# frgfm/Holocron

Measured on AMD Instinct MI355X. Metric: images/sec fwd+bwd+AdaBelief, RepVGG-A0 bs256/GPU 224^2, higher is better.
Workload: dtype bf16; 1 GPU; repvgg_a0 bf16 train step (fwd+bwd+AdaBelief), synthetic 224^2, bs=256 per MI355X (BASELINE.json configs[1]), random-init weights, 10 classes, CE label_smoothing 0.1; global_batch=256, parallelism=dp1, mode=weight gradients on a second stream; hipGraph replay of the full step, dump_outputs=/tmp/code/gt15__hip_graft__frgfm__Holocron/driver_out/dump_parent, deterministic=True

## Files before the change

holocron_amd/_lib.py:

```python
import ctypes as C
import os

import torch

_HERE = os.path.dirname(os.path.abspath(__file__))
LIB_PATH = os.environ.get("HC_LIB_PATH") or os.path.join(_HERE, "lib", "libholocron_hip.so")

HC_MAX_TAPS = 12
HC_MT_CHUNK = 8192
HC_STAT_REPLICAS = 128

c_void_p, c_int32, c_int64, c_float, c_double = C.c_void_p, C.c_int32, C.c_int64, C.c_float, C.c_double


class ConvClass(C.Structure):
    _fields_ = [("OHg", c_int32), ("OWg", c_int32), ("oy0", c_int32), ("ox0", c_int32), ("ostep", c_int32),
                ("istep", c_int32), ("ntaps", c_int32), ("tap", c_int32 * HC_MAX_TAPS)]


class ConvDesc(C.Structure):
    _fields_ = [("src0", c_void_p), ("src1", c_void_p), ("wpk", c_void_p), ("dst", c_void_p), ("resid", c_void_p),
                ("stats", c_void_p), ("bias", c_void_p), ("act", c_int32),
                ("N", c_int32), ("IH", c_int32), ("IW", c_int32), ("srcC", c_int32),
                ("OH", c_int32), ("OW", c_int32), ("Cout", c_int32), ("T", c_int32), ("nclass", c_int32),
# ... 160 lines not shown
    "hc_space_to_depth": (c_int32, [c_void_p] * 2 + [c_int32] * 8 + [c_void_p]),
    "hc_leaky_bwd": (c_int32, [c_void_p, c_int32, c_void_p, c_void_p, c_int64, c_int32, c_float, c_void_p]),
    "hc_yolo1_loss_fwd": (c_int32, [c_void_p] * 3 + [c_int32] * 8 + [c_void_p] * 4 + [c_int32] + [c_void_p] * 4),
    "hc_yolo1_loss_bwd": (c_int32, [c_void_p] * 3 + [c_int32] * 8 + [c_void_p] * 4 + [c_int32] + [c_void_p] * 7),
    "hc_yolo1_decode": (c_int32, [c_void_p] * 3 + [c_int32] * 7 + [c_void_p] * 4),
    "hc_yolo_format_fwd": (c_int32, [c_void_p] * 2 + [c_int32] * 7 + [c_void_p] * 5),
    "hc_yolo_format_bwd": (c_int32, [c_void_p] * 3 + [c_int32] * 7 + [c_void_p] * 7),
    "hc_lamb_step": (c_int32, [c_void_p, c_int32, c_void_p, c_void_p, c_void_p, c_int32, c_void_p]),
    "hc_tadam_step": (c_int32, [c_void_p, c_int32, c_void_p, c_void_p, c_void_p, c_void_p, c_void_p, c_void_p, c_int32, c_void_p]),
    "hc_adan_step": (c_int32, [c_void_p, c_void_p, c_int32, c_void_p, c_void_p]),
    "hc_lookahead_sync": (c_int32, [c_void_p, c_int32, c_float, c_void_p]),
    "hc_multi_copy": (c_int32, [C.POINTER(MultiCopyDesc), c_void_p]),
    "hc_msbn_finalize": (c_int32, [C.POINTER(MsbnDesc), c_void_p]),
    "hc_msbn_bwd_finalize": (c_int32, [C.POINTER(MsbnDesc), c_void_p]),
    "hc_msbn_apply": (c_int32, [C.POINTER(MsbnIo), c_void_p, c_void_p, c_void_p, c_int32, c_void_p]),
    "hc_msbn_bwd_reduce": (c_int32, [C.POINTER(MsbnIo), c_void_p, c_int32, c_void_p, c_void_p, c_int32, c_void_p]),
    "hc_msbn_bwd_apply": (c_int32, [C.POINTER(MsbnIo), c_void_p, c_int32, c_void_p, c_void_p, c_int32, c_void_p]),
    "hc_dwrep_dgrad": (c_int32, [c_void_p, c_void_p, c_int32, c_void_p, c_void_p] + [c_int32] * 5 + [c_void_p]),
    "hc_conv_gather": (c_int32, [C.POINTER(ConvDesc), c_void_p]),
    "hc_conv_pointwise_supported": (c_int32, [C.POINTER(ConvDesc)]),
    "hc_conv_pointwise": (c_int32, [C.POINTER(ConvDesc), c_void_p]),
    "hc_conv_small": (c_int32, [C.POINTER(ConvSmallDesc), c_void_p]),
    "hc_conv_small_supported": (c_int32, [C.POINTER(ConvSmallDesc)]),
    "hc_conv_s2_supported": (c_int32, [C.POINTER(ConvS2Desc)]),
    "hc_conv_s2_fwd": (c_int32, [C.POINTER(ConvS2Desc), c_void_p]),
    "hc_conv_s2_dgrad_supported": (c_int32, [C.POINTER(ConvS2DgradDesc)]),
    "hc_conv_s2_dgrad": (c_int32, [C.POINTER(ConvS2DgradDesc), c_void_p]),
    "hc_conv_s2_stem_wgrad_ws_bytes": (c_int64, []),
    "hc_conv_s2_stem_wgrad": (c_int32, [c_void_p] * 6 + [c_int32] * 4 + [c_void_p]),
    "hc_conv_wgrad_ws_bytes": (c_int64, [C.POINTER(WgradDesc)]),
    "hc_conv_wgrad": (c_int32, [C.POINTER(WgradDesc), c_void_p]),
    "hc_conv_wgrad_group_supported": (c_int32, [C.POINTER(WgradGroupDesc)]),
    "hc_conv_wgrad_group_ws_bytes": (c_int64, [C.POINTER(WgradGroupDesc)]),
    "hc_conv_wgrad_group": (c_int32, [C.POINTER(WgradGroupDesc), c_void_p]),
    "hc_rep_wgrad_supported": (c_int32, [C.POINTER(RepWgradDesc)]),
    "hc_rep_wgrad_ws_bytes": (c_int64, [C.POINTER(RepWgradDesc)]),
    "hc_rep_wgrad_plan": (c_int32, [C.POINTER(RepWgradDesc), c_void_p]),
    "hc_rep_wgrad": (c_int32, [C.POINTER(RepWgradDesc), c_void_p]),
    "hc_pack_conv_weight": (c_int32, [c_void_p, c_void_p] + [c_int32] * 7 + [c_void_p]),
    "hc_pack_conv_weights_multi": (c_int32, [c_void_p, c_int32, c_int64, c_void_p]),
    "hc_nchw_to_nhwc_bf16": (c_int32, [c_void_p, c_void_p] + [c_int32] * 5 + [c_void_p]),
    "hc_nhwc_bf16_to_nchw": (c_int32, [c_void_p, c_void_p] + [c_int32] * 5 + [c_void_p]),
    "hc_im2col_small": (c_int32, [c_void_p, c_void_p] + [c_int32] * 11 + [c_void_p]),
    "hc_unpack_im2col_grad": (c_int32, [c_void_p, c_void_p] + [c_int32] * 6 + [c_void_p]),
    "hc_rep_bn_finalize": (c_int32, [C.POINTER(RepBnDesc), c_void_p]),
    "hc_rep_apply": (c_int32, [c_void_p] * 6 + [c_int64, c_int32, c_int32, c_void_p]),
# ... 152 lines not shown
```

holocron_amd/build.py:

```python
import os
import subprocess
import sys
from concurrent.futures import ThreadPoolExecutor

ROOT = os.path.dirname(os.path.abspath(__file__))
CSRC = os.path.join(ROOT, "csrc")
LIBDIR = os.path.join(ROOT, "lib")
LIB = os.path.join(LIBDIR, "libholocron_hip.so")
HIPCC = os.environ.get("HIPCC", "/opt/rocm/bin/hipcc")
ARCH = "gfx950"

SOURCES = {
    "conv_gather.hip": ["-mllvm", "-pragma-unroll-threshold=131072"],
    "conv_pointwise.hip": [],
    "conv_small.hip": [],
    "conv_wgrad.hip": [],
    "conv_wgrad_tr.hip": [],
    "conv_wgrad_dma.hip": [],
    "conv_wgrad_rep.hip": [],
    "conv_rows.hip": [],
    "conv_rows48.hip": [],
    "conv_s2.hip": [],
    "rep_bn.hip": [],
    "optim.hip": [],
    "nhwc_ops.hip": [],
    "dwconv.hip": [],
    "se_mlp.hip": [],
    "mobileone.hip": [],
    "pointwise.hip": ["-ffp-contract=off"],
    "losses.hip": ["-ffp-contract=off"],
    "yolo.hip": ["-ffp-contract=off"],
}
COMMON = ["--offload-arch=" + ARCH, "-O3", "-std=c++17", "-fPIC", "-Wno-unused-result"]


def _deps():
    hdrs = [os.path.join(CSRC, "common.h"), os.path.join(ROOT, "..", "include", "holocron_hip.h")]
    return max(os.path.getmtime(h) for h in hdrs)


def _compile(item):
    src, flags = item
    obj = os.path.join(LIBDIR, src.replace(".hip", ".o"))
    srcp = os.path.join(CSRC, src)
    if os.path.exists(obj) and os.path.getmtime(obj) >= max(os.path.getmtime(srcp), _deps()):
        return obj, False
    cmd = [HIPCC] + COMMON + flags + ["-c", srcp, "-o", obj]
    r = subprocess.run(cmd, capture_output=True, text=True)
    if r.returncode != 0:
        raise RuntimeError("hipcc failed for %s:\n%s\n%s" % (src, r.stdout, r.stderr))
    return obj, True


def build(force: bool = False, verbose: bool = False) -> str:
    os.makedirs(LIBDIR, exist_ok=True)
    if force:
        for f in os.listdir(LIBDIR):
            if f.endswith(".o") or f.endswith(".so"):
                os.remove(os.path.join(LIBDIR, f))
    with ThreadPoolExecutor(max_workers=min(8, len(SOURCES))) as ex:
# ... 16 lines not shown
```

holocron_amd/csrc/conv_rows.hip:

```cpp
#include <type_traits>
#include "common.h"
#include "../../include/holocron_hip.h"

namespace crw {

constexpr int NT = 512, UR = 7;

struct Args {
    hc_conv_small_desc d;
    int reps;
    int delay;
};

template <int C, int W>
struct Geo {
    static constexpr int CK = C / 32;
    static constexpr int PSC = C / 8 + 1;
    static constexpr int PS = PSC * 16;
    static constexpr int SEGW = W > 0 ? (W + 15) / 16 : (C >= 192 ? 1 : 2);
    static constexpr int WMAX = W > 0 ? W : 16 * SEGW;
    static constexpr int WW = WMAX + 1;
    static constexpr int NSLOT = (UR + 2) * WW + 1;
    static constexpr int NDMA = (NSLOT * PS + 1023) / 1024;
    static constexpr int WIN = NDMA * 1024;
    static constexpr int CWN = 4 / SEGW;
    static constexpr int SMEM = 2 * WIN + 64 + 1024;
    static constexpr int S3 = 9 * CK, S1 = CK, S = S3 + S1;
    static_assert(C == 48 * CWN, "one wave = 48 output channels");
    static_assert(CK % 3 == 0, "three rotating weight register sets per tap");
    static_assert((PS / 8) % 4 == 2, "pixel pitch must be 2 x odd 8-byte units");
    static_assert(SMEM <= 160 * 1024, "LDS budget");
};

__device__ __forceinline__ void dma16s(const u32x4 rsrc, unsigned lds_off, unsigned voff, unsigned soff) {
    asm volatile("s_mov_b32 m0, %0\n\ts_nop 0\n\tbuffer_load_dwordx4 %1, %2, %3 offen lds" ::"s"(lds_off), "v"(voff), "s"(rsrc), "s"(soff)
                 : "memory");
}
__device__ __forceinline__ u32x4 uniform_rsrc(const void* p, unsigned bytes) {
    const unsigned long long v = reinterpret_cast<unsigned long long>(p);
    u32x4 r;
    r[0] = __builtin_amdgcn_readfirstlane((unsigned)v);
    r[1] = __builtin_amdgcn_readfirstlane((unsigned)(v >> 32) & 0xffffu);
    r[2] = __builtin_amdgcn_readfirstlane(bytes);
    r[3] = 0x00020000u;
    return r;
}
__device__ __forceinline__ bf16x8 frag2(const char* lo_p, const char* hi_p) {
    const u32x2 lo = *reinterpret_cast<const u32x2*>(lo_p), hi = *reinterpret_cast<const u32x2*>(hi_p);
    const u32x4 v = {lo[0], lo[1], hi[0], hi[1]};
    return __builtin_bit_cast(bf16x8, v);
}
__device__ __forceinline__ float row16_sum(float v) {
    v += __builtin_bit_cast(float, __builtin_amdgcn_update_dpp(0, __builtin_bit_cast(int, v), 0x128, 0xf, 0xf, false));
    v += __builtin_bit_cast(float, __builtin_amdgcn_update_dpp(0, __builtin_bit_cast(int, v), 0x124, 0xf, 0xf, false));
    v += __builtin_bit_cast(float, __builtin_amdgcn_update_dpp(0, __builtin_bit_cast(int, v), 0x122, 0xf, 0xf, false));
    v += __builtin_bit_cast(float, __builtin_amdgcn_update_dpp(0, __builtin_bit_cast(int, v), 0x121, 0xf, 0xf, false));
    return v;
}

template <int C, int W, int MODE, int DBG>
__global__ __launch_bounds__(NT, 1) void conv_rows_kernel(const Args a) {
    using G = Geo<C, W>;
    extern __shared__ __attribute__((aligned(1024))) char smem[];
    const hc_conv_small_desc& d = a.d;
    constexpr int CK = G::CK, PS = G::PS, WW = G::WW, S3 = G::S3, S1 = G::S1, S = G::S;
    const int tid = threadIdx.x, lane = tid & 63;
    const int wid = __builtin_amdgcn_readfirstlane(tid >> 6);
    const int team = wid >> 2, w4 = wid & 3;
    const int cw = w4 % G::CWN, pw = w4 / G::CWN;
    const int H = d.H, UPI = W > 0 ? H / UR : (H + UR - 1) / UR;
    const int Wr = W > 0 ? W : d.W;
    const int n = blockIdx.x;
    const unsigned lds0 = hc_lds_addr(smem);
    const int px = lane & 15, g = lane >> 4;
    const int col = 16 * pw + px;
    const bool col_ok = col < Wr;
    const int region = team * G::WIN;
    int* cnt = reinterpret_cast<int*>(smem + 2 * G::WIN) + team * 8;
    int gen = 0;
    if (tid < 16) reinterpret_cast<int*>(smem + 2 * G::WIN)[tid] = 0;
    __syncthreads();
    auto team_sync = [&]() __attribute__((always_inline)) {
        asm volatile("s_waitcnt vmcnt(0) lgkmcnt(0)" ::: "memory");
        gen += 4;
        if (lane == 0) __hip_atomic_fetch_add(cnt, 1, __ATOMIC_RELAXED, __HIP_MEMORY_SCOPE_WORKGROUP);
        while (__hip_atomic_load(cnt, __ATOMIC_RELAXED, __HIP_MEMORY_SCOPE_WORKGROUP) < gen) __builtin_amdgcn_s_sleep(1);
        asm volatile("" ::: "memory");
    };
    if (team == 1)
        for (int i = 0; i < a.delay; ++i) __builtin_amdgcn_s_sleep(64);

    const unsigned act_bytes = (unsigned)d.N * H * Wr * C * 2u;
    const u32x4 rsA = uniform_rsrc(d.srcA, act_bytes);
    const u32x4 rsB = uniform_rsrc(MODE == 1 ? d.srcB : d.srcA, act_bytes);
    const __amdgpu_buffer_rsrc_t rsw = make_rsrc(d.w3, (unsigned)(S * C * 64));

    const unsigned wl = (unsigned)((48 * cw + (lane & 15)) * 64 + g * 16);
    u32x4 af[3][3];
    auto load_a = [&](int buf, int s) __attribute__((always_inline)) {
        if (DBG & 4) return;
        const int ps = MODE == 0 ? (s < S1 ? S3 + s : s - S1) : s;
#pragma unroll
        for (int f = 0; f < 3; ++f) af[buf][f] = buf_load16(rsw, wl, (unsigned)(ps * (C * 64) + f * 1024));
    };

    auto stage_window = [&](const u32x4 rs, int row0, int j0, int j1) __attribute__((always_inline)) {
        if (DBG & 8) return;
        const unsigned img = (unsigned)n * (unsigned)(H * Wr * C * 2);
        for (int j = j0 + w4; j < j1; j += 4) {
            const int J = j * 64 + lane;
            const int slot = J / G::PSC, c = J - slot * G::PSC;
            const int r = slot / WW, x = slot - r * WW;
            const int ih = row0 - 1 + r;
            const bool ok = c < G::PSC - 1 && slot < G::NSLOT && x >= 1 && (W > 0 || x <= Wr) && ih >= 0 && ih < H;
            const unsigned off = img + (unsigned)((ih * Wr + x - 1) * C * 2 + c * 16);
            hc_dma16(rs, lds0 + (unsigned)(region + j * 1024), ok ? off : HC_OOB);
        }
    };

    const int vb = region + (WW + col + 1) * PS + g * 8;
    bf16x8 bfr[2][UR];
    auto load_b = [&](int buf, int bofs) __attribute__((always_inline)) {
        if (DBG & 2) return;
        const char* sb = smem + vb + bofs;
#pragma unroll
        for (int i = 0; i < UR; ++i) bfr[buf][i] = frag2(sb + i * WW * PS, sb + i * WW * PS + 32);
    };

    f32x4 acc[3][UR];
    auto zero_acc = [&]() __attribute__((always_inline)) {
#pragma unroll
        for (int f = 0; f < 3; ++f)
#pragma unroll
            for (int i = 0; i < UR; ++i) acc[f][i] = f32x4{0.f, 0.f, 0.f, 0.f};
    };
    auto mfma_step = [&](int ab, int bb) __attribute__((always_inline)) {
#pragma unroll
        for (int i = 0; i < UR; ++i)
#pragma unroll
// ... 36 lines not shown
        for (int k = 0; k < 2; ++k)
#pragma unroll
            for (int e = 0; e < 12; ++e) st[k][e] = 0.f;
#pragma unroll
        for (int i = 0; i < UR; ++i) {
            const bool ok = col_ok && (W > 0 || row0 + i < H);
            const int rr = W > 0 ? row0 + i : (ok ? row0 + i : 0);
            const size_t e0 = img + (size_t)(rr * Wr + (col_ok ? col : 0)) * C + cbase;
            bf16_t* op = reinterpret_cast<bf16_t*>(outp) + e0;
            const bf16_t* rp = residp != nullptr ? reinterpret_cast<const bf16_t*>(residp) + e0 : nullptr;
            u32x2 pk[3];
#pragma unroll
            for (int f = 0; f < 3; ++f) {
                f32x4 v = acc[f][i];
                const int cofs = f < 2 ? 4 * f : 32 - 4 * g;
                if (stats != nullptr) {
#pragma unroll
                    for (int e = 0; e < 4; ++e) {
                        const float x = ok ? v[e] : 0.f;
                        st[0][f * 4 + e] += x;
                        st[1][f * 4 + e] += x * x;
                    }
                }
                if (MODE == 1 && rp != nullptr && ok) {
                    const u32x2 rv = *reinterpret_cast<const u32x2*>(rp + cofs);
                    v[0] += bf16lo(rv[0]); v[1] += bf16hi(rv[0]); v[2] += bf16lo(rv[1]); v[3] += bf16hi(rv[1]);
                }
                pk[f] = u32x2{pack_bf16x2(v[0], v[1]), pack_bf16x2(v[2], v[3])};
                if (MODE == 1 && ok) *reinterpret_cast<u32x2*>(op + cofs) = pk[f];
            }
            if (MODE == 0 && ok) {
                *reinterpret_cast<u32x4*>(op) = u32x4{pk[0][0], pk[0][1], pk[1][0], pk[1][1]};
                *reinterpret_cast<u32x2*>(op + 32 - 4 * g) = pk[2];
            }
        }
        if (stats != nullptr) {
            float* rep = stats + (size_t)((blockIdx.x * 8 + wid) % a.reps) * 2 * C + cbase;
#pragma unroll
            for (int k = 0; k < 2; ++k) {
                float mine = 0.f;
#pragma unroll
                for (int e = 0; e < 12; ++e) {
                    const float x = row16_sum(st[k][e]);
                    mine = px == e ? x : mine;
                }
                if (px < 12) atomicAdd(rep + k * C + (px < 8 ? px : 24 - 4 * g + px), mine);
            }
        }
    };

    for (int u = team; u < UPI; u += 2) {
        const int row0 = u * UR;
        if (u >= 2) team_sync();
        stage_window(rsA, row0, 0, G::NDMA);
        team_sync();
        load_a(0, 0);
        load_a(1, 1);
        zero_acc();
        auto tap_ofs = [&](int tap) __attribute__((always_inline)) { return tap < 9 ? ((tap / 3 - 1) * WW + (tap % 3 - 1)) * PS : 0; };
        if (MODE == 0) {
            load_b(0, 0);
            tap_block(std::integral_constant<int, 0>{}, 0, S, 0, tap_ofs(0), true);
            epilogue(d.out1, d.stats1, nullptr, row0);
            zero_acc();
#pragma nounroll
            for (int tap = 0; tap < 8; tap += 2) {
                const int o0 = tap_ofs(tap), o1 = tap_ofs(tap + 1), o2 = tap_ofs(tap + 2);
                tap_block(std::integral_constant<int, (CK & 1)>{}, (tap + 1) * CK, S, o0, o1, true);
                tap_block(std::integral_constant<int, 0>{}, (tap + 2) * CK, S, o1, o2, true);
            }
            tap_block(std::integral_constant<int, (CK & 1)>{}, 9 * CK, S, tap_ofs(8), 0, false);
            epilogue(d.out3, d.stats3, nullptr, row0);
        } else {
            load_b(0, (-WW - 1) * PS);
#pragma nounroll
            for (int tap = 0; tap < 8; tap += 2) {
                const int o0 = tap_ofs(tap), o1 = tap_ofs(tap + 1), o2 = tap_ofs(tap + 2);
// ... 1 lines not shown
                tap_block(std::integral_constant<int, (CK & 1)>{}, (tap + 1) * CK, S, o1, o2, true);
            }
            tap_block(std::integral_constant<int, 0>{}, 8 * CK, S, tap_ofs(8), 0, false);
            team_sync();
            stage_window(rsB, row0, (WW * PS) / 1024, (8 * WW * PS + PS + 1023) / 1024);
            team_sync();
            load_b(S3 & 1, 0);
            tap_block(std::integral_constant<int, (S3 & 1)>{}, S3, S, 0, 0, false);
            epilogue(d.out3, nullptr, d.resid, row0);
        }
    }
}

template <int C, int W>
bool shape_ok(const hc_conv_small_desc& d) {
    if (W == 0)
        return d.C == C && d.Cout == C && d.W >= 1 && d.W <= Geo<C, 0>::WMAX && d.H >= 1 && d.N >= 1 &&
               (double)d.N * d.H * d.W * C * 2.0 < 2147483000.0;
    return d.C == C && d.Cout == C && d.W == W && d.H >= 2 * UR && d.H % (2 * UR) == 0 && d.H <= 56 && d.N >= 1 &&
           (double)d.N * d.H * d.W * C * 2.0 < 2147483000.0;
}

template <int C, int W, int MODE, int DBG>
void launch1(const Args& a, hipStream_t st) {
    auto kern = conv_rows_kernel<C, W, MODE, DBG>;
    constexpr int smem = Geo<C, W>::SMEM;
    static bool attr_set = false;
    if (!attr_set) {
        (void)hipFuncSetAttribute(reinterpret_cast<const void*>(kern), hipFuncAttributeMaxDynamicSharedMemorySize, smem);
        attr_set = true;
    }
    hipLaunchKernelGGL(kern, dim3(a.d.N), dim3(NT), smem, st, a);
}

template <int C, int W>
void launch(const Args& a, hipStream_t st) {
    static const int dbg = getenv("HC_CRW_DBG") ? atoi(getenv("HC_CRW_DBG")) : 0;
    const bool dg = (a.d.mode & 1) == 1;
#define CRW_CASE(k) case k: if (dg) launch1<C, W, 1, k>(a, st); else launch1<C, W, 0, k>(a, st); break;
    switch (dbg) {
        CRW_CASE(1) CRW_CASE(2) CRW_CASE(3) CRW_CASE(4) CRW_CASE(7) CRW_CASE(8) CRW_CASE(16) CRW_CASE(24) CRW_CASE(31)
        default: if (dg) launch1<C, W, 1, 0>(a, st); else launch1<C, W, 0, 0>(a, st); break;
    }
#undef CRW_CASE
}

}

bool hc_conv_rows_supported(const hc_conv_small_desc& d) {
    static const bool on = [] { const char* e = getenv("HC_CONV_ROWS"); return e == nullptr || atoi(e) != 0; }();
    if (!on || (d.mode & HC_CONV_SMALL_ROWS_IMAGE) == 0 || (d.mode & ~(HC_CONV_SMALL_ROWS_IMAGE | 1)) != 0) return false;
    constexpr bool any = true;
    if (crw::shape_ok<192, 14>(d) || crw::shape_ok<96, 28>(d)) return true;
    return any && (crw::shape_ok<192, 0>(d) || crw::shape_ok<96, 0>(d));
}
int hc_conv_rows_launch(const hc_conv_small_desc& d, hipStream_t st) {
    if (!hc_conv_rows_supported(d)) return HC_ERR_ARG;
    const bool dg = (d.mode & 1) == 1;
    if (d.srcA == nullptr || d.w3 == nullptr || d.out3 == nullptr) return HC_ERR_ARG;
    if (!dg && d.out1 == nullptr) return HC_ERR_ARG;
    if (dg && d.srcB == nullptr) return HC_ERR_ARG;
    if (!dg && (d.stats3 == nullptr) != (d.stats1 == nullptr)) return HC_ERR_ARG;
    crw::Args a;
    a.d = d;
    a.reps = hc_get_stat_replicas();
    constexpr int delay = 0;
    a.delay = delay;
    if (crw::shape_ok<192, 14>(d)) crw::launch<192, 14>(a, st);
    else if (crw::shape_ok<96, 28>(d)) crw::launch<96, 28>(a, st);
    else if (d.C == 192) { if (dg) crw::launch1<192, 0, 1, 0>(a, st); else crw::launch1<192, 0, 0, 0>(a, st); }
    else { if (dg) crw::launch1<96, 0, 1, 0>(a, st); else crw::launch1<96, 0, 0, 0>(a, st); }
    return hc_launch_status();
}
```

holocron_amd/csrc/rep_bn.hip:

```cpp
#include "common.h"
#include "../../include/holocron_hip.h"
#include <stdlib.h>

namespace {

constexpr int EW_THREADS = 256;

struct EwGrid {
    int blocks;
};
inline int ew_blocks(long nchunks, int cg, int cpt_default = 8) {
    int a = cg, b = EW_THREADS;
    while (b) { int t = a % b; a = b; b = t; }
    const int unit = cg / a;
    const int cpt = cpt_default;
    long want = nchunks / (EW_THREADS * cpt);
    constexpr long fl = 1024;
    long floor_blocks = nchunks / (EW_THREADS * 2);
    if (floor_blocks > fl) floor_blocks = fl;
    if (want < floor_blocks) want = floor_blocks;
    if (want > 2048) want = 2048;
    if (want < 1) want = 1;
    long k = (want + unit - 1) / unit;
    return (int)(k * unit);
}

__device__ __forceinline__ void unpack8(const u32x4 v, float (&f)[8]) {
#pragma unroll
    for (int i = 0; i < 4; ++i) { f[2 * i] = bf16lo(v[i]); f[2 * i + 1] = bf16hi(v[i]); }
}
__device__ __forceinline__ u32x4 pack8(const float (&f)[8]) {
    u32x4 v;
#pragma unroll
    for (int i = 0; i < 4; ++i) v[i] = pack_bf16x2(f[2 * i], f[2 * i + 1]);
    return v;
}
__device__ __forceinline__ void load8f(const float* p, float (&f)[8]) {
    const f32x4 a = *reinterpret_cast<const f32x4*>(p), b = *reinterpret_cast<const f32x4*>(p + 4);
#pragma unroll
    for (int i = 0; i < 4; ++i) { f[i] = a[i]; f[4 + i] = b[i]; }
}

template <bool NT>
__device__ __forceinline__ u32x4 ld16(const u32x4* p) {
    return NT ? __builtin_nontemporal_load(p) : *p;
}
template <bool NT>
__device__ __forceinline__ void st16(u32x4* p, const u32x4 v) {
    if (NT) __builtin_nontemporal_store(v, p);
    else *p = v;
}
static inline bool ba_streaming(long nchunks) { return nchunks * 16 >= 200L * 1000000L; }
static inline bool ew_streaming(long nchunks) {
    constexpr long thr = 48;
    return thr >= 0 && nchunks * 16 >= thr * 1000000L;
}

template <int S>
__device__ __forceinline__ void block_reduce_flush(const float (&v)[S][8], int cg, int C, float* __restrict__ dst,
                                                   float* __restrict__ lds, int nsum) {
    constexpr int STR = S * 8 + 1;
    const int tid = threadIdx.x;
#pragma unroll
    for (int k = 0; k < S; ++k)
#pragma unroll
// ... 87 lines not shown
                invstd = rsqrtf(var + d.eps);
                if (d.running_mean[b] != nullptr) {
                    const float unb = d.count > 1 ? var * (cnt / (cnt - 1.f)) : var;
                    d.running_mean[b][c] = (1.f - d.momentum) * rm[b] + d.momentum * mean;
                    d.running_var[b][c] = (1.f - d.momentum) * rv[b] + d.momentum * unb;
                }
                if (c == 0 && d.num_batches_tracked[b] != nullptr) d.num_batches_tracked[b][0] += 1;
            } else {
                mean = rm[b];
                invstd = rsqrtf(rv[b] + d.eps);
            }
            a = gam[b] * invstd;
            shift += bet[b] - a * mean;
        }
        d.coef[b * d.C + c] = a;
        if (d.save != nullptr) {
            d.save[(2 * b) * d.C + c] = mean;
            d.save[(2 * b + 1) * d.C + c] = invstd;
        }
    }
    d.coef[3 * d.C + c] = shift;
}

template <bool HAS_ID>
__device__ __forceinline__ float rep_preact(float a3, float f3, float a1, float f1, float a0, float f0, float sh) {
    float z = __builtin_fmaf(a1, f1, sh);
    if (HAS_ID) z = __builtin_fmaf(a0, f0, z);
    return __builtin_fmaf(a3, f3, z);
}
template <bool HAS_ID, bool STATS, bool NT>
__global__ __launch_bounds__(EW_THREADS) void rep_apply_kernel(const u32x4* __restrict__ y3, const u32x4* __restrict__ y1,
                                                               const u32x4* __restrict__ x, const float* __restrict__ coef,
                                                               u32x4* __restrict__ out, float* __restrict__ out_stats,
                                                               long nchunks, int C, int act, const int reps) {
    extern __shared__ float sred[];
    const int cg = C / 8;
    const long gtid = (long)blockIdx.x * EW_THREADS + threadIdx.x;
    const long stride = (long)gridDim.x * EW_THREADS;
    const int c0 = (int)(gtid % cg) * 8;
    float a3[8], a1[8], a0[8], sh[8];
    load8f(coef + c0, a3);
    load8f(coef + C + c0, a1);
    if (HAS_ID) load8f(coef + 2 * C + c0, a0);
    load8f(coef + 3 * C + c0, sh);
    float sv[2][8];
#pragma unroll
    for (int i = 0; i < 8; ++i) sv[0][i] = sv[1][i] = 0.f;
    for (long q = gtid; q < nchunks; q += stride) {
        float f3[8], f1[8], f0[8], o[8];
        unpack8(ld16<NT>(y3 + q), f3);
        unpack8(ld16<NT>(y1 + q), f1);
        if (HAS_ID) unpack8(ld16<NT>(x + q), f0);
// ... 169 lines not shown
    const long stride = (long)gridDim.x * EW_THREADS;
    const int c0 = (int)(gtid % cg) * 8;
    float a3[8], a1[8], a0[8], sh[8];
    if (ZMASK) {
        load8f(coef + c0, a3);
        load8f(coef + C + c0, a1);
        if (HAS_ID) load8f(coef + 2 * C + c0, a0);
        load8f(coef + 3 * C + c0, sh);
    }
    float A3[8], B3[8], C3[8], A1[8], B1[8], C1[8], A0[8], B0[8], C0[8];
    load8f(bc + 0 * C + c0, A3); load8f(bc + 1 * C + c0, B3); load8f(bc + 2 * C + c0, C3);
    load8f(bc + 3 * C + c0, A1); load8f(bc + 4 * C + c0, B1); load8f(bc + 5 * C + c0, C1);
    if (HAS_ID) { load8f(bc + 6 * C + c0, A0); load8f(bc + 7 * C + c0, B0); load8f(bc + 8 * C + c0, C0); }
    for (long q = gtid; q < nchunks; q += stride) {
        float fg[8], fo[8], f3[8], f1[8], f0[8], o3[8], o1[8], o0[8];
        unpack8(ld16<NT>(g + q), fg);
        if (!ZMASK) unpack8(ld16<NT>(out + q), fo);
        unpack8(ld16<NT>(y3 + q), f3);
        unpack8(ld16<NT>(y1 + q), f1);
        if (HAS_ID) unpack8(ld16<NT>(x + q), f0);
#pragma unroll
        for (int i = 0; i < 8; ++i) {
            if (ZMASK) fo[i] = act == 1 ? rep_preact<HAS_ID>(a3[i], f3[i], a1[i], f1[i], HAS_ID ? a0[i] : 0.f, HAS_ID ? f0[i] : 0.f, sh[i]) : 1.f;
            const float dz = fo[i] > 0.f ? fg[i] : 0.f;
            o3[i] = __builtin_fmaf(A3[i], dz, __builtin_fmaf(B3[i], f3[i], C3[i]));
            o1[i] = __builtin_fmaf(A1[i], dz, __builtin_fmaf(B1[i], f1[i], C1[i]));
            if (HAS_ID) o0[i] = __builtin_fmaf(A0[i], dz, __builtin_fmaf(B0[i], f0[i], C0[i]));
        }
        st16<NT>(dy3 + q, pack8(o3));
        st16<NT>(dy1 + q, pack8(o1));
        if (HAS_ID) st16<NT>(dxid + q, pack8(o0));
    }
}

__device__ __forceinline__ float act_fwd(float v, int act, float slope) {
    switch (act) {
        case 1: return v > 0.f ? v : 0.f;
        case 2: { const float t = fminf(fmaxf(v + 2.f, 0.f), 2.f); return 0.5f * v * t; }
        case 3: return v > 0.f ? v : slope * v;
        case 4: {
            const float e = __expf(fminf(v, 20.f)), n = e * (e + 2.f);
            return v * n * __builtin_amdgcn_rcpf(n + 2.f);
        }
        case 5: return v * __builtin_amdgcn_rcpf(1.f + __expf(-v));
        case 6: return fminf(fmaxf(v, 0.f), 6.f);
        default: return v;
    }
}
__device__ __forceinline__ float act_bwd(float v, int act, float slope) {
    switch (act) {
// ... 1030 lines not shown
```

holocron_amd/nn/repblock_op.py:

```python
import ctypes as C

import os

import torch

from .. import _lib
from .._lib import ConvS2Desc, ConvS2DgradDesc, PackItem, RepBnBwdDesc, RepBnDesc, StemBwdDesc, StemDesc, check, ptr, stream
from ..ops import conv as cv

STEM_KPAD = 32


class ZeroPool:

    def __init__(self):
        self.buf = None
        self.used = 0
        self.high = 0
        self.depth = 0
        self.gen = 0
        self.retired = []
        self.graph_users = 0
        self.buf_captured = False

    def _retire(self):
        if self.buf is not None and self.buf_captured:
            self.retired.append(self.buf)
        self.buf, self.buf_captured = None, False

    def release_retired(self):
        self.graph_users = max(0, self.graph_users - 1)
        if self.graph_users == 0:
            self.retired = []
# ... 294 lines not shown
    return y3, y1


def block_dgrad(st, dy3, dy1, dxid, w3, w1, geom):
    N, Cin, H, W, Cout = geom
    _, _, dg, _, sdg = st.descs(N, Cin, H, W, Cout)
    wpd = st.ensure_packed(w3, w1)[2]
    dx = cv.empty_cl(N, Cin, H, W, dy3.device)
    s2g = st.desc[(N, Cin, H, W, Cout)][7]
    if s2g is not None:
        if dxid is not None:
            raise _lib.HipError("stride-2 data gradient: a stride-2 RepBlock has no identity branch")
        s2g.dy3, s2g.dy1, s2g.wimg, s2g.dx = ptr(dy3), ptr(dy1), ptr(st.s2_dimg), ptr(dx)
        with cv.profiled("conv_s2", 2.0 * N * dy3.shape[2] * dy3.shape[3] * Cout * 10 * Cin, dx.numel() * 2.0 + 2 * dy3.numel() * 2.0):
            check(_lib.load().hc_conv_s2_dgrad(C.byref(s2g), stream()), "hc_conv_s2_dgrad")
        return dx
    if sdg is not None:
        cv.launch_conv_small_dgrad(sdg, dy3, dy1, wpd, dx, resid=dxid)
    else:
        cv.launch_conv(dg, dy3, wpd, dx, src1=dy1, resid=dxid)
    return dx


def block_wgrad(st, src, dy3, dy1, w3, w1, geom, stem_cin=None, defer=False):
    N, Cin, H, W, Cout = geom
    lib = _lib.load()
    npix = dy3.shape[0] * dy3.shape[2] * dy3.shape[3]
    if stem_cin is not None and src.dtype == torch.float32:
        dw3 = torch.empty_like(w3, dtype=torch.float32)
        dw1 = torch.empty_like(w1, dtype=torch.float32)
        ws = torch.empty((int(lib.hc_conv_s2_stem_wgrad_ws_bytes()),), dtype=torch.uint8, device=src.device)
        with cv.profiled("conv_wgrad", 2.0 * npix * Cout * 10 * stem_cin, src.numel() * 4.0 + 2 * dy3.numel() * 2.0):
            rc = lib.hc_conv_s2_stem_wgrad(ptr(src), ptr(dy3), ptr(dy1), ptr(dw3), ptr(dw1), ptr(ws), N, H, W, 0, stream())
        if rc == 0:
            return dw3, dw1
        src = cv.im2col_small(src, 3, 3, st.stride, 1, STEM_KPAD)
    if stem_cin is not None:
        K = STEM_KPAD
        dwc3 = cv.conv_wgrad(src, dy3, K, Cout, 1, 1, 1, 0, flops=2.0 * npix * Cout * 9 * stem_cin)
        dwc1 = cv.conv_wgrad(src, dy1, K, Cout, 1, 1, 1, 0, flops=2.0 * npix * Cout * stem_cin)
        dw3 = torch.empty_like(w3, dtype=torch.float32)
        check(lib.hc_unpack_im2col_grad(ptr(dwc3), ptr(dw3), Cout, stem_cin, 3, 3, K, 0, stream()), "hc_unpack_im2col_grad")
        dw1 = dwc1.view(Cout, K)[:, 4 * stem_cin:5 * stem_cin].reshape(Cout, stem_cin, 1, 1).contiguous()
        return dw3, dw1
    fused = cv.rep_block_wgrad(src, dy3, dy1, w3, w1, st.stride, defer=defer)
    if fused is not None:
# ... 132 lines not shown
            return (None, dw3, dw1, dgam[0], dbet[0], dgam[1], dbet[1], None, None, None, None)
        red = POOL.claim(ctx.red, ctx.red_gen, (_lib.stat_replicas(), 4, Cout), dev)
        ctx.red = None
        with cv.profiled("bn_elementwise", 0.0, tb * (4 if st.identity else 3)):
            check(lib.hc_rep_bwd_reduce_z(ptr(g), ptr(coef), act, ptr(y3), ptr(y1), ptr(xid), ptr(red), npix, Cout, stream()),
                  "hc_rep_bwd_reduce_z")
        nb = 3 if st.identity else 2
        dgam = torch.empty((3, Cout), dtype=torch.float32, device=dev)
        dbet = torch.empty((3, Cout), dtype=torch.float32, device=dev)
        bcoef = torch.empty((9, Cout), dtype=torch.float32, device=dev)
        d = RepBnBwdDesc()
        d.red, d.save, d.bcoef = ptr(red), ptr(save), ptr(bcoef)
        gam = (g3, g1, g0)
        for b in range(3):
            live = b < nb
            d.gamma[b] = ptr(gam[b]) if live else None
            d.dgamma[b] = ptr(dgam[b]) if live else None
            d.dbeta[b] = ptr(dbet[b]) if live else None
        d.C, d.count, d.has_identity, d.accumulate = Cout, npix, 1 if st.identity else 0, 0
        d.frozen = 0 if ctx.was_training else 1
        with cv.profiled("bn_finalize", 0.0, 0.0):
            check(lib.hc_rep_bn_bwd_finalize(C.byref(d), stream()), "hc_rep_bn_bwd_finalize")

        dy3 = torch.empty_like(y3)
        dy1 = torch.empty_like(y1)
        dxid = torch.empty_like(src) if st.identity else None
        with cv.profiled("bn_elementwise", 0.0, tb * (7 if st.identity else 5)):
            check(lib.hc_rep_bwd_apply_z(ptr(g), ptr(coef), act, ptr(y3), ptr(y1), ptr(xid), ptr(bcoef), ptr(dy3), ptr(dy1),
                                         ptr(dxid), npix, Cout, stream()), "hc_rep_bwd_apply_z")

        dx = None
        geom = (N, Cin, H, W, Cout)
        if ctx.needs_input_grad[0]:
            if ctx.stem:
                raise NotImplementedError("input gradient of the im2col stem path")
            dx = block_dgrad(st, dy3, dy1, dxid, w3, w1, geom)

        with cv.side_stream_for_wgrad((w3, w1), (src, dy3, dy1)) as side:
            dw3, dw1 = block_wgrad(st, src, dy3, dy1, w3, w1, geom, Cin if ctx.stem else None, defer=True)
            side.produced(dw3, dw1)
        return (dx, dw3, dw1, dgam[0], dbet[0], dgam[1], dbet[1],
                dgam[2] if st.identity else None, dbet[2] if st.identity else None, None, None)


def rep_block_forward(x, w3, w1, bn3, bn1, bn0, st, relu=True):
    st.bn = [(bn3.running_mean, bn3.running_var, bn3.num_batches_tracked),
             (bn1.running_mean, bn1.running_var, bn1.num_batches_tracked),
             (bn0.running_mean, bn0.running_var, bn0.num_batches_tracked) if bn0 is not None else (None, None, None)]
    st.eps = bn3.eps
    st.momentum = 0.1 if bn3.momentum is None else bn3.momentum
    st.training = bn3.training
    if bn1.training != bn3.training or (bn0 is not None and bn0.training != bn3.training):
        raise NotImplementedError("RepBlock (HIP): the BatchNorm layers of one block must all be in the same mode (freeze the "
                                  "whole block, e.g. freeze_model(model, 'features.2.1'), not a single branch)")
    out = RepBlockFn.apply(x, w3, w1, bn3.weight, bn3.bias, bn1.weight, bn1.bias,
                           bn0.weight if bn0 is not None else None, bn0.bias if bn0 is not None else None, st, relu)
    if st.last_out_stats is not None:
        out._hc_stats = st.last_out_stats
        st.last_out_stats = None
# ... 2 lines not shown
```

include/holocron_hip.h:

```cpp
#ifndef HOLOCRON_HIP_H
#define HOLOCRON_HIP_H
#include <stdint.h>
#ifdef __cplusplus
extern "C" {
#endif

typedef void* hc_stream_t;

#define HC_MAX_TAPS 12
#define HC_STAT_REPLICAS 128
#define HC_STAT_REPLICAS_DETERMINISTIC 32768
int hc_set_deterministic(int on);
int hc_get_deterministic(void);
int hc_get_stat_replicas(void);

typedef struct {
    int32_t OHg, OWg, oy0, ox0, ostep, istep, ntaps;
    int32_t tap[HC_MAX_TAPS];
} hc_conv_class;
#define HC_TAP(dy, dx, src, wt) \
    ((int32_t)(((uint32_t)(dy) & 0xffu) | (((uint32_t)(dx) & 0xffu) << 8) | ((uint32_t)(src) << 16) | ((uint32_t)(wt) << 24)))

typedef struct {
    const void* src0;
// ... 20 lines not shown
    float act_slope;
    int32_t resid_after_act;
} hc_conv_desc;
int hc_conv_gather(const hc_conv_desc* d, hc_stream_t stream);
int hc_conv_pointwise_supported(const hc_conv_desc* d);
int hc_conv_pointwise(const hc_conv_desc* d, hc_stream_t stream);

#define HC_CONV_SMALL_ROWS_IMAGE 4
typedef struct {
    const void* srcA;
    const void* srcB;
    const void* w3;
    const void* w1;
    void* out3;
    void* out1;
    const void* resid;
    float* stats3;
    float* stats1;
    int32_t w3_rstride, w1_rstride;
    int32_t N, H, W, C, Cout, mode;
} hc_conv_small_desc;
int hc_conv_small(const hc_conv_small_desc* d, hc_stream_t stream);
int hc_conv_small_supported(const hc_conv_small_desc* d);

typedef struct {
    const void* x;
    const void* w3img;
    const void* w1img;
    void* y3;
    void* y1;
    float* stats3;
    float* stats1;
    int32_t N, H, W, Cin, Cout, x_nchw_f32;
} hc_conv_s2_desc;
int hc_conv_s2_supported(const hc_conv_s2_desc* d);
int hc_conv_s2_fwd(const hc_conv_s2_desc* d, hc_stream_t stream);
typedef struct {
    const void* dy3;
    const void* dy1;
    const void* wimg;
    void* dx;
    int32_t N, H, W, Cin, Cout;
} hc_conv_s2_dgrad_desc;
int hc_conv_s2_dgrad_supported(const hc_conv_s2_dgrad_desc* d);
int hc_conv_s2_dgrad(const hc_conv_s2_dgrad_desc* d, hc_stream_t stream);
int64_t hc_conv_s2_stem_wgrad_ws_bytes(void);
// ... 452 lines not shown
```

Before: 26150 images/sec.

## Fuse RepVGG BN-backward elementwise into the row-conv dgrad kernel prologue

```diff
diff --git a/holocron_amd/_lib.py b/holocron_amd/_lib.py
--- a/holocron_amd/_lib.py
+++ b/holocron_amd/_lib.py
@@ -206,6 +206,8 @@
     "hc_conv_pointwise": (c_int32, [C.POINTER(ConvDesc), c_void_p]),
     "hc_conv_small": (c_int32, [C.POINTER(ConvSmallDesc), c_void_p]),
     "hc_conv_small_supported": (c_int32, [C.POINTER(ConvSmallDesc)]),
+    "hc_conv_rows_fused_bwd_supported": (c_int32, [C.POINTER(ConvSmallDesc)]),
+    "hc_conv_rows_fused_bwd": (c_int32, [C.POINTER(ConvSmallDesc), c_void_p, c_void_p, c_int32] + [c_void_p] * 8),
     "hc_conv_s2_supported": (c_int32, [C.POINTER(ConvS2Desc)]),
     "hc_conv_s2_fwd": (c_int32, [C.POINTER(ConvS2Desc), c_void_p]),
     "hc_conv_s2_dgrad_supported": (c_int32, [C.POINTER(ConvS2DgradDesc)]),
diff --git a/holocron_amd/build.py b/holocron_amd/build.py
--- a/holocron_amd/build.py
+++ b/holocron_amd/build.py
@@ -35,7 +35,7 @@
 
 
 def _deps():
-    hdrs = [os.path.join(CSRC, "common.h"), os.path.join(ROOT, "..", "include", "holocron_hip.h")]
+    hdrs = [os.path.join(CSRC, "common.h"), os.path.join(CSRC, "rep_ew.h"), os.path.join(ROOT, "..", "include", "holocron_hip.h")]
     return max(os.path.getmtime(h) for h in hdrs)
 
 
diff --git a/holocron_amd/csrc/conv_rows.hip b/holocron_amd/csrc/conv_rows.hip
--- a/holocron_amd/csrc/conv_rows.hip
+++ b/holocron_amd/csrc/conv_rows.hip
@@ -1,5 +1,6 @@
 #include <type_traits>
 #include "common.h"
+#include "rep_ew.h"
 #include "../../include/holocron_hip.h"
 
 namespace crw {
@@ -10,6 +11,12 @@
     hc_conv_small_desc d;
     int reps;
     int delay;
+};
+struct FusedArgs : Args {
+    const void *g, *y3, *y1, *x;
+    const float *coef, *bcoef;
+    void* dy3;
+    int act;
 };
 
 template <int C, int W>
@@ -36,6 +43,9 @@
     asm volatile("s_mov_b32 m0, %0\n\ts_nop 0\n\tbuffer_load_dwordx4 %1, %2, %3 offen lds" ::"s"(lds_off), "v"(voff), "s"(rsrc), "s"(soff)
                  : "memory");
 }
+__device__ __forceinline__ void dma16_sc1(const u32x4 rsrc, unsigned lds_off, unsigned voff) {
+    asm volatile("s_mov_b32 m0, %0\n\ts_nop 0\n\tbuffer_load_dwordx4 %1, %2, 0 offen sc1 lds" ::"s"(lds_off), "v"(voff), "s"(rsrc) : "memory");
+}
 __device__ __forceinline__ u32x4 uniform_rsrc(const void* p, unsigned bytes) {
     const unsigned long long v = reinterpret_cast<unsigned long long>(p);
     u32x4 r;
@@ -59,7 +69,7 @@
 }
 
 template <int C, int W, int MODE, int DBG>
-__global__ __launch_bounds__(NT, 1) void conv_rows_kernel(const Args a) {
+__global__ __launch_bounds__(NT, 1) void conv_rows_kernel(const std::conditional_t<MODE == 2, FusedArgs, Args> a) {
     using G = Geo<C, W>;
     extern __shared__ __attribute__((aligned(1024))) char smem[];
     const hc_conv_small_desc& d = a.d;
@@ -92,7 +102,7 @@
 
     const unsigned act_bytes = (unsigned)d.N * H * Wr * C * 2u;
     const u32x4 rsA = uniform_rsrc(d.srcA, act_bytes);
-    const u32x4 rsB = uniform_rsrc(MODE == 1 ? d.srcB : d.srcA, act_bytes);
+    const u32x4 rsB = uniform_rsrc(MODE != 0 ? d.srcB : d.srcA, act_bytes);
     const __amdgpu_buffer_rsrc_t rsw = make_rsrc(d.w3, (unsigned)(S * C * 64));
 
     const unsigned wl = (unsigned)((48 * cw + (lane & 15)) * 64 + g * 16);
@@ -114,7 +124,91 @@
             const int ih = row0 - 1 + r;
             const bool ok = c < G::PSC - 1 && slot < G::NSLOT && x >= 1 && (W > 0 || x <= Wr) && ih >= 0 && ih < H;
             const unsigned off = img + (unsigned)((ih * Wr + x - 1) * C * 2 + c * 16);
-            hc_dma16(rs, lds0 + (unsigned)(region + j * 1024), ok ? off : HC_OOB);
+            if (MODE == 2) dma16_sc1(rs, lds0 + (unsigned)(region + j * 1024), ok ? off : HC_OOB);
+            else hc_dma16(rs, lds0 + (unsigned)(region + j * 1024), ok ? off : HC_OOB);
+        }
+    };
+
+    auto fused_prologue = [&](int row0) __attribute__((always_inline)) {
+        if constexpr (MODE == 2) {
+            if (DBG & 32) return;
+            constexpr int CG = C / 8, PPS = 256 / CG, BATCH = 2;
+            for (int j = w4; j < G::NDMA; j += 4) {
+                const int J = j * 64 + lane;
+                const int slot = J / G::PSC, c = J - slot * G::PSC;
+                const int r = slot / WW, x = slot - r * WW;
+                const int ih = row0 - 1 + r;
+                const bool ok = c < G::PSC - 1 && slot < G::NSLOT && x >= 1 && (W > 0 || x <= Wr) && ih >= 0 && ih < H;
+                if (!ok) *reinterpret_cast<u32x4*>(smem + region + J * 16) = u32x4{0u, 0u, 0u, 0u};
+            }
+            const int tt = w4 * 64 + lane;
+            const int pl = tt / CG, chunk = tt - pl * CG;
+            const bool active = pl < PPS;
+            int c0 = chunk * 8;
+            asm volatile("" : "+v"(c0));
+            float a3[8], a1[8], a0[8], sh[8], A3[8], B3[8], C3[8], A1[8], B1[8], C1[8], A0[8], B0[8], C0[8];
+            load8f(a.coef + c0, a3); load8f(a.coef + C + c0, a1); load8f(a.coef + 2 * C + c0, a0); load8f(a.coef + 3 * C + c0, sh);
+            load8f(a.bcoef + 0 * C + c0, A3); load8f(a.bcoef + 1 * C + c0, B3); load8f(a.bcoef + 2 * C + c0, C3);
+            load8f(a.bcoef + 3 * C + c0, A1); load8f(a.bcoef + 4 * C + c0, B1); load8f(a.bcoef + 5 * C + c0, C1);
+            load8f(a.bcoef + 6 * C + c0, A0); load8f(a.bcoef + 7 * C + c0, B0); load8f(a.bcoef + 8 * C + c0, C0);
+            const __amdgpu_buffer_rsrc_t rg = make_rsrc(a.g, act_bytes), r3 = make_rsrc(a.y3, act_bytes), r1 = make_rsrc(a.y1, act_bytes),
+                                         rx = make_rsrc(a.x, act_bytes), rd3 = make_rsrc(a.dy3, act_bytes),
+                                         rd1 = make_rsrc(d.srcB, act_bytes), rd0 = make_rsrc(d.resid, act_bytes);
+            const int HW = H * Wr, NP = (UR + 2) * Wr;
+            const int gp0 = (row0 - 1) * Wr;
+            const int act = a.act;
+            struct Batch { u32x4 vg[BATCH], v3[BATCH], v1[BATCH], vx[BATCH]; unsigned off[BATCH]; };
+            auto request = [&](Batch& q, int pb) __attribute__((always_inline)) {
+#pragma unroll
+                for (int b = 0; b < BATCH; ++b) {
+                    const int p = pb + b * PPS, gp = gp0 + p;
+                    const bool ok = active && p < NP && gp >= 0 && gp < HW;
+                    q.off[b] = ok ? (unsigned)(((n * HW + gp) * CG + chunk) * 16) : HC_OOB;
+                    q.vg[b] = buf_load16(rg, q.off[b]);
+                    q.v3[b] = buf_load16(r3, q.off[b]);
+                    q.v1[b] = buf_load16(r1, q.off[b]);
+                    q.vx[b] = buf_load16(rx, q.off[b]);
+                }
+            };
+            auto finish = [&](const Batch& q, int pb) __attribute__((always_inline)) {
+#pragma unroll
+                for (int b = 0; b < BATCH; ++b) {
+                    const int p = pb + b * PPS;
+                    float fg[8], f3[8], f1[8], f0[8], o3[8], o1[8], o0[8];
+                    unpack8(q.vg[b], fg); unpack8(q.v3[b], f3); unpack8(q.v1[b], f1); unpack8(q.vx[b], f0);
+#pragma unroll
+                    for (int i = 0; i < 8; ++i) {
+                        const float fo = act == 1 ? rep_preact<true>(a3[i], f3[i], a1[i], f1[i], a0[i], f0[i], sh[i]) : 1.f;
+                        const float dz = rep_bwd_dz(fo, fg[i]);
+                        o3[i] = rep_bwd_branch(A3[i], dz, B3[i], f3[i], C3[i]);
+                        o1[i] = rep_bwd_branch(A1[i], dz, B1[i], f1[i], C1[i]);
+                        o0[i] = rep_bwd_branch(A0[i], dz, B0[i], f0[i], C0[i]);
+                    }
+                    const u32x4 p3 = pack8(o3);
+                    if (q.off[b] != HC_OOB) {
+                        const int r = p / Wr, x = p - r * Wr;
+                        *reinterpret_cast<u32x4*>(smem + region + (r * WW + x + 1) * PS + chunk * 16) = p3;
+                    }
+                    const unsigned so = (p >= Wr && p < (UR + 1) * Wr) ? q.off[b] : HC_OOB;
+                    __builtin_amdgcn_raw_buffer_store_b128(p3, rd3, so, 0, 0);
+                    __builtin_amdgcn_raw_buffer_store_b128(pack8(o1), rd1, so, 0, 0);
+                    __builtin_amdgcn_raw_buffer_store_b128(pack8(o0), rd0, so, 0, 0);
+                }
+            };
+            constexpr int STEP = BATCH * PPS;
+            Batch q0, q1;
+            request(q0, pl);
+#pragma nounroll
+            for (int pb = pl; pb < NP + pl; pb += 2 * STEP) {
+                request(q1, pb + STEP);
+                __builtin_amdgcn_sched_barrier(0);
+                finish(q0, pb);
+                __builtin_amdgcn_sched_barrier(0);
+                request(q0, pb + 2 * STEP);
+                __builtin_amdgcn_sched_barrier(0);
+                finish(q1, pb + STEP);
+                __builtin_amdgcn_sched_barrier(0);
+            }
         }
     };
 
@@ -197,12 +291,14 @@
                         st[1][f * 4 + e] += x * x;
                     }
                 }
-                if (MODE == 1 && rp != nullptr && ok) {
-                    const u32x2 rv = *reinterpret_cast<const u32x2*>(rp + cofs);
+                if (MODE != 0 && rp != nullptr && ok) {
+                    const u32x2 rv = MODE == 2 ? __builtin_bit_cast(u32x2, __hip_atomic_load(reinterpret_cast<const unsigned long long*>(rp + cofs),
+                                                                                             __ATOMIC_RELAXED, __HIP_MEMORY_SCOPE_AGENT))
+                                               : *reinterpret_cast<const u32x2*>(rp + cofs);
                     v[0] += bf16lo(rv[0]); v[1] += bf16hi(rv[0]); v[2] += bf16lo(rv[1]); v[3] += bf16hi(rv[1]);
                 }
                 pk[f] = u32x2{pack_bf16x2(v[0], v[1]), pack_bf16x2(v[2], v[3])};
-                if (MODE == 1 && ok) *reinterpret_cast<u32x2*>(op + cofs) = pk[f];
+                if (MODE != 0 && ok) *reinterpret_cast<u32x2*>(op + cofs) = pk[f];
             }
             if (MODE == 0 && ok) {
                 *reinterpret_cast<u32x4*>(op) = u32x4{pk[0][0], pk[0][1], pk[1][0], pk[1][1]};
@@ -227,7 +323,8 @@
     for (int u = team; u < UPI; u += 2) {
         const int row0 = u * UR;
         if (u >= 2) team_sync();
-        stage_window(rsA, row0, 0, G::NDMA);
+        if (MODE == 2) fused_prologue(row0);
+        else stage_window(rsA, row0, 0, G::NDMA);
         team_sync();
         load_a(0, 0);
         load_a(1, 1);
@@ -275,7 +372,7 @@
 }
 
 template <int C, int W, int MODE, int DBG>
-void launch1(const Args& a, hipStream_t st) {
+void launch1(const std::conditional_t<MODE == 2, FusedArgs, Args>& a, hipStream_t st) {
     auto kern = conv_rows_kernel<C, W, MODE, DBG>;
     constexpr int smem = Geo<C, W>::SMEM;
     static bool attr_set = false;
@@ -294,6 +391,17 @@
     switch (dbg) {
         CRW_CASE(1) CRW_CASE(2) CRW_CASE(3) CRW_CASE(4) CRW_CASE(7) CRW_CASE(8) CRW_CASE(16) CRW_CASE(24) CRW_CASE(31)
         default: if (dg) launch1<C, W, 1, 0>(a, st); else launch1<C, W, 0, 0>(a, st); break;
+    }
+#undef CRW_CASE
+}
+
+template <int C, int W>
+void launch_fused(const FusedArgs& a, hipStream_t st) {
+    static const int dbg = getenv("HC_CRW_DBG") ? atoi(getenv("HC_CRW_DBG")) : 0;
+#define CRW_CASE(k) case k: launch1<C, W, 2, k>(a, st); break;
+    switch (dbg) {
+        CRW_CASE(1) CRW_CASE(2) CRW_CASE(3) CRW_CASE(4) CRW_CASE(7) CRW_CASE(8) CRW_CASE(16) CRW_CASE(24) CRW_CASE(31) CRW_CASE(32)
+        default: launch1<C, W, 2, 0>(a, st); break;
     }
 #undef CRW_CASE
 }
@@ -325,3 +433,30 @@
     else { if (dg) crw::launch1<96, 0, 1, 0>(a, st); else crw::launch1<96, 0, 0, 0>(a, st); }
     return hc_launch_status();
 }
+
+extern "C" int hc_conv_rows_fused_bwd_supported(const hc_conv_small_desc* dp) {
+    return dp != nullptr && dp->mode == (HC_CONV_SMALL_ROWS_IMAGE | 1) && hc_conv_rows_supported(*dp) ? 1 : 0;
+}
+extern "C" int hc_conv_rows_fused_bwd(const hc_conv_small_desc* dp, const void* g, const float* coef, int32_t act, const void* y3,
+                                      const void* y1, const void* x, const float* bcoef, void* dy3, void* dy1, void* dxid,
+                                      hc_stream_t stream) {
+    if (!hc_conv_rows_fused_bwd_supported(dp)) return HC_ERR_ARG;
+    if (dp->w3 == nullptr || dp->out3 == nullptr || g == nullptr || coef == nullptr || y3 == nullptr || y1 == nullptr || x == nullptr ||
+        bcoef == nullptr || dy3 == nullptr || dy1 == nullptr || dxid == nullptr || (act != 0 && act != 1))
+        return HC_ERR_ARG;
+    const hc_conv_small_desc& d = *dp;
+    hipStream_t st = (hipStream_t)stream;
+    crw::FusedArgs a;
+    a.d = d;
+    a.d.srcA = dy3;
+    a.d.srcB = dy1;
+    a.d.resid = dxid;
+    a.reps = hc_get_stat_replicas();
+    a.delay = 0;
+    a.g = g; a.y3 = y3; a.y1 = y1; a.x = x; a.coef = coef; a.bcoef = bcoef; a.dy3 = dy3; a.act = act;
+    if (crw::shape_ok<192, 14>(d)) crw::launch_fused<192, 14>(a, st);
+    else if (crw::shape_ok<96, 28>(d)) crw::launch_fused<96, 28>(a, st);
+    else if (d.C == 192) crw::launch1<192, 0, 2, 0>(a, st);
+    else crw::launch1<96, 0, 2, 0>(a, st);
+    return hc_launch_status();
+}
diff --git a/holocron_amd/csrc/rep_bn.hip b/holocron_amd/csrc/rep_bn.hip
--- a/holocron_amd/csrc/rep_bn.hip
+++ b/holocron_amd/csrc/rep_bn.hip
@@ -1,4 +1,5 @@
 #include "common.h"
+#include "rep_ew.h"
 #include "../../include/holocron_hip.h"
 #include <stdlib.h>
 
@@ -25,22 +26,6 @@
     return (int)(k * unit);
 }
 
-__device__ __forceinline__ void unpack8(const u32x4 v, float (&f)[8]) {
-#pragma unroll
-    for (int i = 0; i < 4; ++i) { f[2 * i] = bf16lo(v[i]); f[2 * i + 1] = bf16hi(v[i]); }
-}
-__device__ __forceinline__ u32x4 pack8(const float (&f)[8]) {
-    u32x4 v;
-#pragma unroll
-    for (int i = 0; i < 4; ++i) v[i] = pack_bf16x2(f[2 * i], f[2 * i + 1]);
-    return v;
-}
-__device__ __forceinline__ void load8f(const float* p, float (&f)[8]) {
-    const f32x4 a = *reinterpret_cast<const f32x4*>(p), b = *reinterpret_cast<const f32x4*>(p + 4);
-#pragma unroll
-    for (int i = 0; i < 4; ++i) { f[i] = a[i]; f[4 + i] = b[i]; }
-}
-
 template <bool NT>
 __device__ __forceinline__ u32x4 ld16(const u32x4* p) {
     return NT ? __builtin_nontemporal_load(p) : *p;
@@ -174,12 +159,6 @@
     d.coef[3 * d.C + c] = shift;
 }
 
-template <bool HAS_ID>
-__device__ __forceinline__ float rep_preact(float a3, float f3, float a1, float f1, float a0, float f0, float sh) {
-    float z = __builtin_fmaf(a1, f1, sh);
-    if (HAS_ID) z = __builtin_fmaf(a0, f0, z);
-    return __builtin_fmaf(a3, f3, z);
-}
 template <bool HAS_ID, bool STATS, bool NT>
 __global__ __launch_bounds__(EW_THREADS) void rep_apply_kernel(const u32x4* __restrict__ y3, const u32x4* __restrict__ y1,
                                                                const u32x4* __restrict__ x, const float* __restrict__ coef,
@@ -395,10 +374,10 @@
 #pragma unroll
         for (int i = 0; i < 8; ++i) {
             if (ZMASK) fo[i] = act == 1 ? rep_preact<HAS_ID>(a3[i], f3[i], a1[i], f1[i], HAS_ID ? a0[i] : 0.f, HAS_ID ? f0[i] : 0.f, sh[i]) : 1.f;
-            const float dz = fo[i] > 0.f ? fg[i] : 0.f;
-            o3[i] = __builtin_fmaf(A3[i], dz, __builtin_fmaf(B3[i], f3[i], C3[i]));
-            o1[i] = __builtin_fmaf(A1[i], dz, __builtin_fmaf(B1[i], f1[i], C1[i]));
-            if (HAS_ID) o0[i] = __builtin_fmaf(A0[i], dz, __builtin_fmaf(B0[i], f0[i], C0[i]));
+            const float dz = rep_bwd_dz(fo[i], fg[i]);
+            o3[i] = rep_bwd_branch(A3[i], dz, B3[i], f3[i], C3[i]);
+            o1[i] = rep_bwd_branch(A1[i], dz, B1[i], f1[i], C1[i]);
+            if (HAS_ID) o0[i] = rep_bwd_branch(A0[i], dz, B0[i], f0[i], C0[i]);
         }
         st16<NT>(dy3 + q, pack8(o3));
         st16<NT>(dy1 + q, pack8(o1));
diff --git a/holocron_amd/csrc/rep_ew.h b/holocron_amd/csrc/rep_ew.h
--- /dev/null
+++ b/holocron_amd/csrc/rep_ew.h
@@ -0,0 +1,30 @@
+#pragma once
+#include "common.h"
+
+__device__ __forceinline__ void unpack8(const u32x4 v, float (&f)[8]) {
+#pragma unroll
+    for (int i = 0; i < 4; ++i) { f[2 * i] = bf16lo(v[i]); f[2 * i + 1] = bf16hi(v[i]); }
+}
+__device__ __forceinline__ u32x4 pack8(const float (&f)[8]) {
+    u32x4 v;
+#pragma unroll
+    for (int i = 0; i < 4; ++i) v[i] = pack_bf16x2(f[2 * i], f[2 * i + 1]);
+    return v;
+}
+__device__ __forceinline__ void load8f(const float* p, float (&f)[8]) {
+    const f32x4 a = *reinterpret_cast<const f32x4*>(p), b = *reinterpret_cast<const f32x4*>(p + 4);
+#pragma unroll
+    for (int i = 0; i < 4; ++i) { f[i] = a[i]; f[4 + i] = b[i]; }
+}
+
+template <bool HAS_ID>
+__device__ __forceinline__ float rep_preact(float a3, float f3, float a1, float f1, float a0, float f0, float sh) {
+    float z = __builtin_fmaf(a1, f1, sh);
+    if (HAS_ID) z = __builtin_fmaf(a0, f0, z);
+    return __builtin_fmaf(a3, f3, z);
+}
+
+__device__ __forceinline__ float rep_bwd_dz(float fo, float g) { return fo > 0.f ? g : 0.f; }
+__device__ __forceinline__ float rep_bwd_branch(float A, float dz, float B, float y, float Cc) {
+    return __builtin_fmaf(A, dz, __builtin_fmaf(B, y, Cc));
+}
diff --git a/holocron_amd/nn/repblock_op.py b/holocron_amd/nn/repblock_op.py
--- a/holocron_amd/nn/repblock_op.py
+++ b/holocron_amd/nn/repblock_op.py
@@ -9,6 +9,7 @@
 from ..ops import conv as cv
 
 STEM_KPAD = 32
+FUSED_BWD = os.environ.get("HC_REP_FUSED_BWD", "1") != "0"
 
 
 class ZeroPool:
@@ -349,6 +350,25 @@
     return dx
 
 
+def fused_dgrad_desc(st, geom):
+    N, Cin, H, W, Cout = geom
+    sdg = st.descs(N, Cin, H, W, Cout)[4]
+    if sdg is None or not st.rows_image[1] or Cin != Cout or not _lib.load().hc_conv_rows_fused_bwd_supported(C.byref(sdg)):
+        return None
+    return sdg
+
+
+def block_dgrad_fused(st, sdg, g, coef, act, y3, y1, x, bcoef, w3, w1, bufs=None):
+    wpd = st.ensure_packed(w3, w1)[2]
+    dy3, dy1, dxid, dx = bufs if bufs is not None else (torch.empty_like(y3), torch.empty_like(y1), torch.empty_like(x), torch.empty_like(x))
+    sdg.srcA, sdg.srcB, sdg.resid, sdg.w3, sdg.w1, sdg.out3, sdg.out1, sdg.stats3, sdg.stats1 = None, None, None, ptr(wpd), None, ptr(dx), None, None, None
+    tb = x.numel() * 2.0
+    with cv.profiled("conv_rows", 2.0 * sdg.N * sdg.H * sdg.W * sdg.Cout * 10 * sdg.C, 8 * tb):
+        check(_lib.load().hc_conv_rows_fused_bwd(C.byref(sdg), ptr(g), ptr(coef), act, ptr(y3), ptr(y1), ptr(x), ptr(bcoef), ptr(dy3),
+                                                 ptr(dy1), ptr(dxid), stream()), "hc_conv_rows_fused_bwd")
+    return dy3, dy1, dxid, dx
+
+
 def block_wgrad(st, src, dy3, dy1, w3, w1, geom, stem_cin=None, defer=False):
     N, Cin, H, W, Cout = geom
     lib = _lib.load()
@@ -527,19 +547,22 @@
         with cv.profiled("bn_finalize", 0.0, 0.0):
             check(lib.hc_rep_bn_bwd_finalize(C.byref(d), stream()), "hc_rep_bn_bwd_finalize")
 
-        dy3 = torch.empty_like(y3)
-        dy1 = torch.empty_like(y1)
-        dxid = torch.empty_like(src) if st.identity else None
-        with cv.profiled("bn_elementwise", 0.0, tb * (7 if st.identity else 5)):
-            check(lib.hc_rep_bwd_apply_z(ptr(g), ptr(coef), act, ptr(y3), ptr(y1), ptr(xid), ptr(bcoef), ptr(dy3), ptr(dy1),
-                                         ptr(dxid), npix, Cout, stream()), "hc_rep_bwd_apply_z")
-
         dx = None
         geom = (N, Cin, H, W, Cout)
-        if ctx.needs_input_grad[0]:
-            if ctx.stem:
-                raise NotImplementedError("input gradient of the im2col stem path")
-            dx = block_dgrad(st, dy3, dy1, dxid, w3, w1, geom)
+        fdg = fused_dgrad_desc(st, geom) if (FUSED_BWD and st.identity and ctx.needs_input_grad[0] and not ctx.stem) else None
+        if fdg is not None:
+            dy3, dy1, dxid, dx = block_dgrad_fused(st, fdg, g, coef, act, y3, y1, src, bcoef, w3, w1)
+        else:
+            dy3 = torch.empty_like(y3)
+            dy1 = torch.empty_like(y1)
+            dxid = torch.empty_like(src) if st.identity else None
+            with cv.profiled("bn_elementwise", 0.0, tb * (7 if st.identity else 5)):
+                check(lib.hc_rep_bwd_apply_z(ptr(g), ptr(coef), act, ptr(y3), ptr(y1), ptr(xid), ptr(bcoef), ptr(dy3), ptr(dy1),
+                                             ptr(dxid), npix, Cout, stream()), "hc_rep_bwd_apply_z")
+            if ctx.needs_input_grad[0]:
+                if ctx.stem:
+                    raise NotImplementedError("input gradient of the im2col stem path")
+                dx = block_dgrad(st, dy3, dy1, dxid, w3, w1, geom)
 
         with cv.side_stream_for_wgrad((w3, w1), (src, dy3, dy1)) as side:
             dw3, dw1 = block_wgrad(st, src, dy3, dy1, w3, w1, geom, Cin if ctx.stem else None, defer=True)
diff --git a/include/holocron_hip.h b/include/holocron_hip.h
--- a/include/holocron_hip.h
+++ b/include/holocron_hip.h
@@ -66,6 +66,9 @@
 } hc_conv_small_desc;
 int hc_conv_small(const hc_conv_small_desc* d, hc_stream_t stream);
 int hc_conv_small_supported(const hc_conv_small_desc* d);
+int hc_conv_rows_fused_bwd_supported(const hc_conv_small_desc* d);
+int hc_conv_rows_fused_bwd(const hc_conv_small_desc* d, const void* g, const float* coef, int32_t act, const void* y3, const void* y1,
+                           const void* x, const float* bcoef, void* dy3, void* dy1, void* dxid, hc_stream_t stream);
 
 typedef struct {
     const void* x;
```

Result: faster. 26620 images/sec (median of 6 runs) (+1.8%).
